# adeyemiadeoye/SelfConcordantSmoothOptimization.jl

Measured on AMD Instinct MI355X. Metric: iterate!() iterations/sec + achieved HBM GB/s, ProxGGNSCORE n=1M m=16k, higher is better.
Workload: dtype f64

## Files before the change

### selfconcordantsmoothoptimization.jl_amd/csrc/gram.hip

```cpp
#include <algorithm>
#include <cstdlib>
#include <type_traits>
#include <vector>

#include "common.h"

namespace scs {

}
#include "gram_strip.h"
namespace scs {

#define LDS_BARRIER()                                          \
  do {                                                         \
    asm volatile("s_waitcnt lgkmcnt(0)" ::: "memory");         \
    __builtin_amdgcn_s_barrier();                              \
    asm volatile("" ::: "memory");                             \
  } while (0)

__device__ __forceinline__ int bnd_claim(unsigned* ctr, int ntiles) {
  const int q8 = ntiles / 8, r8 = ntiles % 8;
  const int x0 = (int)((unsigned)__builtin_amdgcn_s_getreg((15 << 11) | 20) & 7u);
  for (int d = 0; d < 8; ++d) {
    const int x = (x0 + d) & 7, len = q8 + (x < r8 ? 1 : 0);
    if (len == 0) continue;
// ... 443 lines not shown
}

void gram_tile_list(int nb, int2* out, int* ntiles) {
  const int S = 8;
  const int nsb = (nb + S - 1) / S;
  int t = 0;
  for (int sbi = 0; sbi < nsb; ++sbi)
    for (int sbj = 0; sbj <= sbi; ++sbj)
      for (int i = sbi * S; i < (sbi + 1) * S && i < nb; ++i)
        for (int j = sbj * S; j < (sbj + 1) * S && j < nb; ++j)
          if (i >= j) out[t++] = make_int2(i, j);
  *ntiles = t;
}

void gram_tile_list_tall(int nb, int2* out, int* ntiles) {
  const int nbi = nb / 2, SI = 4, SJ = 8;
  int t = 0;
  for (int sbi = 0; sbi < (nbi + SI - 1) / SI; ++sbi)
    for (int sbj = 0; sbj <= sbi; ++sbj)
      for (int I = sbi * SI; I < (sbi + 1) * SI && I < nbi; ++I)
        for (int j = sbj * SJ; j < (sbj + 1) * SJ && j < nb; ++j)
          if (j <= 2 * I + 1) out[t++] = make_int2(I, j);
  *ntiles = t;
}

void gram_tile_list_rowmajor(int nb, int2* out) {
  int t = 0;
  for (int i = 0; i < nb; ++i)
    for (int j = 0; j <= i; ++j) out[t++] = make_int2(i, j);
}

hipError_t gram_launch_gen(const double* A1, int64_t lda1, const double* A2, int64_t lda2, const double* w,
                           int64_t k0, int64_t k1, const int2* tiles, int ntiles, double* G, int64_t ldg, int flags,
                           hipStream_t st);

template <int PIPE, int TI = 2, bool CM = false, bool AV = false, bool BND = false>
__global__ __launch_bounds__(128 * TI, (TI == 2 ? 2 : 1)) void gram_sia_kernel(
    const double* __restrict__ A, int64_t S, const double* __restrict__ w, int64_t k0, int64_t Nk,
// ... 12 lines not shown
    const int4* __restrict__ work, int seglen, int nsplit, double* __restrict__ P,
    const double* __restrict__ v, double* __restrict__ VP, int64_t vps, unsigned* __restrict__ scnt, int sob) {
  constexpr int PIPE = 1;
  constexpr bool CM = false, BND = false;
  const double* const A2 = nullptr;
  const int64_t S2 = 0;
#include "gram_sia_body.h"
}

static int env_int(const char* name, int dflt) {
  const char* e = getenv(name);
  return e ? atoi(e) : dflt;
}
int gram_sia_mode() {
  static const int v = env_int("SCS_GRAM_SIA", 1);
  return v;
}
int gram_tall_mode() {
  static const int v = env_int("SCS_GRAM_GLDS", 3);
  return v;
}

int gram_fuse_ok(int tall) {
  const char* e = getenv("SCS_GRAM_FUSE");
  const int mode = e ? atoi(e) : 1;
  if (mode == 0 || (!tall && mode < 2)) return 0;
  return tall ? gram_tall_mode() == 3 : gram_sia_mode() == 1;
}

__global__ void gram_vfinal_kernel(const double* __restrict__ VP, int npiece, int64_t vps, int64_t m,
                                   double* __restrict__ out) {
  const int64_t f = (int64_t)blockIdx.x * blockDim.x + threadIdx.x;
  if (f >= m) return;
  double s = VP[f];
  for (int p = 1; p < npiece; ++p) s += VP[(int64_t)p * vps + f];
  out[f] = s;
}

hipError_t gram_vfinal_launch(const double* VP, int npiece, int64_t vps, int64_t m, double* out, hipStream_t st) {
  hipLaunchKernelGGL(gram_vfinal_kernel, dim3((unsigned)((m + 255) / 256)), dim3(256), 0, st, VP, npiece, vps, m, out);
  return hipGetLastError();
}

static thread_local const char* g_main_name = "";
const char* gram_main_kernel_name() { return g_main_name; }

hipError_t gram_launch(const void* Av, int a32, int64_t lda, const double* w, int64_t Nk, const int2* tiles,
                       int ntiles, double* G, int64_t ldg, int packed, int tall, hipStream_t st, const double* v,
                       double* VP, int64_t vps) {
  if (ntiles <= 0) return hipSuccess;
  const int flags = ((packed & 1) ? GRAM_PACKED : GRAM_UPPER) | ((packed & 2) ? GRAM_ACCUMULATE : 0);
  if (v && !gram_fuse_ok(tall)) return hipErrorInvalidValue;
  if (a32) {
    const float* A = (const float*)Av;
    if (tall && v) {
      g_main_name = "gram_sia_ta_kernel<float, 4, true>";
      hipLaunchKernelGGL((gram_sia_ta_kernel<float, 4, true>), dim3(ntiles), dim3(512), 0, st, A, lda, w, (int64_t)0,
                         Nk, tiles, ntiles, G, ldg, flags, nullptr, 0, 0, nullptr, v, VP, vps, nullptr, 0);
    } else if (v) {
      g_main_name = "gram_sia_ta_kernel<float, 2, true>";
// ... 3 lines not shown
      g_main_name = "gram_sia_ta_kernel<float, 4, false>";
      hipLaunchKernelGGL((gram_sia_ta_kernel<float, 4, false>), dim3(ntiles), dim3(512), 0, st, A, lda, w, (int64_t)0,
                         Nk, tiles, ntiles, G, ldg, flags, nullptr, 0, 0, nullptr, nullptr, nullptr, (int64_t)0,
                         nullptr, 0);
    } else {
      g_main_name = "gram_sia_ta_kernel<float, 2, false>";
      hipLaunchKernelGGL((gram_sia_ta_kernel<float, 2, false>), dim3(ntiles), dim3(256), 0, st, A, lda, w, (int64_t)0,
                         Nk, tiles, ntiles, G, ldg, flags, nullptr, 0, 0, nullptr, nullptr, nullptr, (int64_t)0,
                         nullptr, 0);
    }
    return hipGetLastError();
  }
  const double* A = (const double*)Av;
  if (v) {
    if (tall) {
      g_main_name = "gram_sia_kernel<1, 4, false, true, false>";
      hipLaunchKernelGGL((gram_sia_kernel<1, 4, false, true>), dim3(ntiles), dim3(512), 0, st, A, lda, w, (int64_t)0,
                         Nk, tiles, ntiles, G, ldg, flags, nullptr, 0, 0, nullptr, v, VP, vps, nullptr, 0, nullptr, (int64_t)0);
    } else {
      g_main_name = "gram_sia_kernel<1, 2, false, true, false>";
      hipLaunchKernelGGL((gram_sia_kernel<1, 2, false, true>), dim3(ntiles), dim3(256), 0, st, A, lda, w, (int64_t)0,
                         Nk, tiles, ntiles, G, ldg, flags, nullptr, 0, 0, nullptr, v, VP, vps, nullptr, 0, nullptr, (int64_t)0);
    }
    return hipGetLastError();
  }
  if (!tall && gram_sia_mode() == 0) {
    g_main_name = "gram_f64_kernel<false, 2, true, false>";
    hipLaunchKernelGGL((gram_f64_kernel<false, 2, true>), dim3(ntiles), dim3(256), 0, st, A, lda, A, lda, w,
                       (int64_t)0, Nk, tiles, ntiles, G, ldg, flags, nullptr, 0, 0, nullptr);
  } else if (!tall) {
    g_main_name = "gram_sia_kernel<1, 2, false, false, false>";
    hipLaunchKernelGGL((gram_sia_kernel<1, 2>), dim3(ntiles), dim3(256), 0, st, A, lda, w, (int64_t)0, Nk, tiles,
                       ntiles, G, ldg, flags, nullptr, 0, 0, nullptr, nullptr, nullptr, (int64_t)0, nullptr, 0, nullptr, (int64_t)0);
  } else if (gram_tall_mode() == 3) {
    g_main_name = "gram_sia_kernel<1, 4, false, false, false>";
    hipLaunchKernelGGL((gram_sia_kernel<1, 4>), dim3(ntiles), dim3(512), 0, st, A, lda, w, (int64_t)0, Nk, tiles,
                       ntiles, G, ldg, flags, nullptr, 0, 0, nullptr, nullptr, nullptr, (int64_t)0, nullptr, 0, nullptr, (int64_t)0);
  } else {
    g_main_name = "gram_glds_kernel<true, 1>";
    hipLaunchKernelGGL((gram_glds_kernel<true, 1>), dim3(ntiles), dim3(512), 0, st, A, lda, A, lda, w, (int64_t)0, Nk,
                       tiles, ntiles, G, ldg, flags, nullptr, 0, 0, nullptr);
  }
  return hipGetLastError();
}

template <int QC>
__global__ __launch_bounds__(256) void gram_small_kernel(const double* __restrict__ A1, int64_t lda1,
                                                         const double* A2, int64_t lda2,
                                                         const double* __restrict__ w, int64_t k0, int64_t Nk,
                                                         const int2* __restrict__ tiles, double* G, int64_t ldg,
                                                         int flags) {
  constexpr int NQ = GT / QC;
// ... 125 lines not shown
                       ntiles, G, ldg, flags, nullptr, 0, 0, nullptr);
  return hipGetLastError();
}

template <int TI>
__global__ void gram_combine_kernel(const double* __restrict__ P, const int4* __restrict__ items, int nsplit,
                                    double* __restrict__ G, int64_t ldg, int packed) {
  constexpr int GTI = 64 * TI;
  const int4 it = items[blockIdx.y];
  for (int e = blockIdx.x * blockDim.x + threadIdx.x; e < GTI * GT; e += gridDim.x * blockDim.x) {
    const int jl = e / GTI, il = e % GTI;
    double sum = 0.0;
    for (int sp = 0; sp < nsplit; ++sp) sum += P[(int64_t)(it.w + sp) * GTI * GT + e];
    double* dst = (packed & 1) ? G + ((int64_t)it.z * (GTI / GT) + il / GT) * GT * GT + jl * GT + (il % GT)
                               : G + ((int64_t)it.x * GTI + il) * ldg + (int64_t)it.y * GT + jl;
    if (packed & 2) *dst += sum;
    else *dst = sum;
  }
}

hipError_t gram_launch_sched(const void* Av, int a32, int64_t lda, const double* w, int64_t Nk, const int4* work,
                             int seglen, int nsplit, const int4* comb, int ncomb, double* P, double* G, int64_t ldg,
                             int packed, int tall, hipStream_t st, const double* v, double* VP, int64_t vps,
                             unsigned* scnt, int sob) {
  const double* A = (const double*)Av;
  if (scnt && !(gram_fuse_ok(tall) || (tall ? gram_tall_mode() == 3 : gram_sia_mode() == 1)))
    return hipErrorInvalidValue;
  const int flags = ((packed & 1) ? GRAM_PACKED : GRAM_UPPER) | ((packed & 2) ? GRAM_ACCUMULATE : 0);
  const int glds = gram_tall_mode();
  if (v && !gram_fuse_ok(tall)) return hipErrorInvalidValue;
// ... 7 lines not shown
      g_main_name = "gram_sia_ta_kernel<float, 2, true>";
      hipLaunchKernelGGL((gram_sia_ta_kernel<float, 2, true>), dim3(8 * seglen), dim3(256), 0, st, Af, lda, w,
                         (int64_t)0, Nk, nullptr, 0, G, ldg, flags, work, seglen, nsplit, P, v, VP, vps, scnt, sob);
    } else if (tall) {
      g_main_name = "gram_sia_ta_kernel<float, 4, false>";
      hipLaunchKernelGGL((gram_sia_ta_kernel<float, 4, false>), dim3(8 * seglen), dim3(512), 0, st, Af, lda, w,
                         (int64_t)0, Nk, nullptr, 0, G, ldg, flags, work, seglen, nsplit, P, nullptr, nullptr,
                         (int64_t)0, scnt, sob);
    } else {
      g_main_name = "gram_sia_ta_kernel<float, 2, false>";
      hipLaunchKernelGGL((gram_sia_ta_kernel<float, 2, false>), dim3(8 * seglen), dim3(256), 0, st, Af, lda, w,
                         (int64_t)0, Nk, nullptr, 0, G, ldg, flags, work, seglen, nsplit, P, nullptr, nullptr,
                         (int64_t)0, scnt, sob);
    }
  } else if (v && tall) {
    g_main_name = "gram_sia_kernel<1, 4, false, true, false>";
    hipLaunchKernelGGL((gram_sia_kernel<1, 4, false, true>), dim3(8 * seglen), dim3(512), 0, st, A, lda, w,
                       (int64_t)0, Nk, nullptr, 0, G, ldg, flags, work, seglen, nsplit, P, v, VP, vps, scnt, sob, nullptr, (int64_t)0);
  } else if (v) {
    g_main_name = "gram_sia_kernel<1, 2, false, true, false>";
    hipLaunchKernelGGL((gram_sia_kernel<1, 2, false, true>), dim3(8 * seglen), dim3(256), 0, st, A, lda, w,
                       (int64_t)0, Nk, nullptr, 0, G, ldg, flags, work, seglen, nsplit, P, v, VP, vps, scnt, sob, nullptr, (int64_t)0);
  } else if (tall && glds == 3) {
    g_main_name = "gram_sia_kernel<1, 4, false, false, false>";
    hipLaunchKernelGGL((gram_sia_kernel<1, 4>), dim3(8 * seglen), dim3(512), 0, st, A, lda, w, (int64_t)0, Nk,
                       nullptr, 0, G, ldg, flags, work, seglen, nsplit, P, nullptr, nullptr, (int64_t)0, scnt, sob, nullptr, (int64_t)0);
  } else if (tall && glds == 2) {
    g_main_name = "gram_glds_kernel<true, 1>";
    hipLaunchKernelGGL((gram_glds_kernel<true, 1>), dim3(8 * seglen), dim3(512), 0, st, A, lda, A, lda, w, (int64_t)0,
                       Nk, nullptr, 0, G, ldg, flags, work, seglen, nsplit, P);
  } else if (tall && glds == 1) {
    g_main_name = "gram_glds_kernel<true, 0>";
    hipLaunchKernelGGL(gram_glds_kernel<true>, dim3(8 * seglen), dim3(512), 0, st, A, lda, A, lda, w, (int64_t)0, Nk,
                       nullptr, 0, G, ldg, flags, work, seglen, nsplit, P);
  } else if (tall) {
    g_main_name = "gram_f64_kernel<false, 4, true, false>";
    hipLaunchKernelGGL((gram_f64_kernel<false, 4, true>), dim3(8 * seglen), dim3(512), 0, st, A, lda, A, lda, w,
                       (int64_t)0, Nk, nullptr, 0, G, ldg, flags, work, seglen, nsplit, P);
  } else if (gram_sia_mode() == 1) {
    g_main_name = "gram_sia_kernel<1, 2, false, false, false>";
    hipLaunchKernelGGL((gram_sia_kernel<1, 2>), dim3(8 * seglen), dim3(256), 0, st, A, lda, w, (int64_t)0, Nk, nullptr,
// ... 57 lines not shown
  int S = 1;
  if (tail_max > 0 && 4 * tail_max < 3 * slots_per_xcd)
    S = std::max(2, std::min(16, slots_per_xcd / tail_max));
  std::vector<std::vector<int4>> seg(8);
  comb.clear();
  int pslot = 0, t0 = 0;
  for (int x = 0; x < 8; ++x) {
    const int n = q + (x < r ? 1 : 0);
    const int tail = (S > 1) ? n % slots_per_xcd : 0;
    for (int i = 0; i < n - tail; ++i) {
      const int2 tl = tiles[t0 + i];
      seg[x].push_back(make_int4(tl.x, tl.y, -1, t0 + i));
    }
    if (diag_first_gti > 0)
      std::stable_partition(seg[x].begin(), seg[x].end(), [&](const int4& it) {
        return it.x == (int)((int64_t)it.y * GT / diag_first_gti);
      });
    for (int i = n - tail; i < n; ++i) {
      const int2 tl = tiles[t0 + i];
      comb.push_back(make_int4(tl.x, tl.y, t0 + i, pslot));
      for (int sp = 0; sp < S; ++sp) seg[x].push_back(make_int4(tl.x, tl.y, sp, pslot + sp));
      pslot += S;
    }
    t0 += n;
  }
  size_t seglen = 0;
  for (auto& v : seg) seglen = std::max(seglen, v.size());
  work.assign(8 * seglen, make_int4(-1, -1, -1, -1));
  for (int x = 0; x < 8; ++x)
    for (size_t i = 0; i < seg[x].size(); ++i) work[x * seglen + i] = seg[x][i];
  *nsplit = S;
// ... 13 lines not shown
```

### selfconcordantsmoothoptimization.jl_amd/csrc/gram_sia_body.h

```cpp
  static_assert(!(AV && CM), "the fused Aᵀv runs on the panel-blocked A only");
  static_assert(!CM || sizeof(TA) == sizeof(double), "column-major operands are fp64");
  constexpr int GTI = 64 * TI;
  constexpr int NT = 128 * TI;
  constexpr int FS = NT / 8;
  constexpr int NTI = 4;
  constexpr int NA = GTI / FS;
  constexpr int NB = GT / FS;
  constexpr int NMM = 2 * NTI * 4;
  constexpr int NRD = NTI + 4;
  constexpr int TAIL = NMM / 4;
  const int packed = flags & GRAM_PACKED, accumulate = flags & GRAM_ACCUMULATE, upper = flags & GRAM_UPPER;
  __shared__ __attribute__((aligned(16))) double lds[(GTI + GT) * GBK];
  const int orig = blockIdx.x;
  const int xcd = orig % 8;
  int bi, bj, tix, part = -1, piece = 0;
  __shared__ int s_claim;
  if constexpr (BND) {
    tix = bnd_first(scnt, (unsigned)sob, ntiles, &s_claim);
    if (tix < 0 || tix >= ntiles) return;
    bi = tiles[tix].x;
    bj = tiles[tix].y;
  } else if (work) {
    const int4 it = work[xcd * seglen + orig / 8];
    if (it.x < 0) return;
    bi = it.x;
    bj = it.y;
    tix = it.w;
// ... 1 lines not shown
      piece = it.z;
      const int64_t L = ((Nk - k0 + (int64_t)nsplit * GBK - 1) / ((int64_t)nsplit * GBK)) * GBK;
      part = it.w;
      k0 = k0 + it.z * L;
      Nk = k0 + L < Nk ? k0 + L : Nk;
      if (Nk < k0) Nk = k0;
    }
  } else {
    const int q8 = ntiles / 8, r8 = ntiles % 8;
    tix = (xcd < r8 ? xcd * (q8 + 1) : r8 * (q8 + 1) + (xcd - r8) * q8) + orig / 8;
    const int2 tl = tiles[tix];
    bi = tl.x;
    bj = tl.y;
  }
bnd_tile:
  int tid_ = threadIdx.x;
  if constexpr (BND) asm volatile("" : "+v"(tid_));
  const int tid = tid_, lane = tid & 63, wid = tid >> 6;
  const int wr = wid >> 1, wc = wid & 1;
  const int sc = tid & 7, sf0 = tid >> 3;
  const int64_t st0 = k0 / GBK;
  const TA* srcA = CM ? A + ((int64_t)bi * GTI + sf0) * S + k0 + 2 * sc
                      : A + ((int64_t)bi * (GTI / GT) * S + st0) * GT * GBK + sf0 * GBK + 2 * sc;
  const TA* B2 = (CM && A2) ? (const TA*)A2 : A;
  const int64_t SB2 = (CM && A2) ? S2 : S;
  const TA* srcB = CM ? B2 + ((int64_t)bj * GT + sf0) * SB2 + k0 + 2 * sc
                      : A + ((int64_t)bj * S + st0) * GT * GBK + sf0 * GBK + 2 * sc;
  const double* srcW = w + k0 + 2 * sc;
  const double* srcV = AV ? v + k0 + 2 * sc : nullptr;
  double* la = lds;
  double* lb = lds + GTI * GBK;
  int woff[NA];
#pragma unroll
  for (int i = 0; i < NA; ++i) {
    const int f = sf0 + FS * i;
    woff[i] = f * GBK + 2 * (sc ^ swz(f));
  }
  typedef typename pair_of<TA>::type PR;
  PR ra[NA], rb[NB];
  v2d rw, rv;
  double av[NB];
#pragma unroll
  for (int i = 0; i < NB; ++i) av[i] = 0.0;
  auto gload = [&](int64_t st, auto fa) {
    constexpr bool FA = decltype(fa)::value;
    if (PIPE == 3 && st >= 2) return;
    if (CM) {
#pragma unroll
      for (int i = 0; i < NA; ++i) ra[i] = *(const PR*)(srcA + st * GBK + (int64_t)FS * i * S);
#pragma unroll
      for (int i = 0; i < NB; ++i) rb[i] = *(const PR*)(srcB + st * GBK + (int64_t)FS * i * SB2);
    } else {
      const int64_t so = st * GT * GBK;
#pragma unroll
      for (int i = 0; i < NA; ++i) {
        const int f = FS * i;
        ra[i] = *(const PR*)(srcA + so + (f >> 7) * S * GT * GBK + (f & 127) * GBK);
      }
#pragma unroll
      for (int i = 0; i < NB; ++i) rb[i] = *(const PR*)(srcB + so + FS * GBK * i);
    }
    rw = *(const v2d*)(srcW + st * GBK);
    if (FA) rv = *(const v2d*)(srcV + st * GBK);
  };
  auto swrite = [&](auto fa) {
    constexpr bool FA = decltype(fa)::value;
#pragma unroll
    for (int i = 0; i < NA; ++i) *(v2d*)(la + woff[i]) = widen(ra[i]);
#pragma unroll
    for (int i = 0; i < NB; ++i) *(v2d*)(lb + woff[i]) = widen(rb[i]) * rw;
    if (FA) {
#pragma unroll
      for (int i = 0; i < NB; ++i) {
        const v2d b = widen(rb[i]);
        av[i] = __builtin_fma(b[1], rv[1], __builtin_fma(b[0], rv[0], av[i]));
      }
    }
  };
  const int fl = lane & 15, g = lane >> 4, s = swz(fl);
  struct Frag {
    v2d a[NTI], b[4];
  };
  auto fread = [&](int p, Frag& F) {
    const int pc = ((4 * p + g) ^ s) * 2;
#pragma unroll
    for (int t = 0; t < NTI; ++t) F.a[t] = *(const v2d*)(la + (wr * 64 + 16 * t + fl) * GBK + pc);
#pragma unroll
    for (int t = 0; t < 4; ++t) F.b[t] = *(const v2d*)(lb + (wc * 64 + 16 * t + fl) * GBK + pc);
  };
  v4d acc[NTI][4];
#pragma unroll
  for (int i = 0; i < NTI; ++i)
#pragma unroll
    for (int j = 0; j < 4; ++j) acc[i][j] = (v4d){0.0, 0.0, 0.0, 0.0};
  auto mm = [&](const Frag& F, int n0, int n1) {
#pragma unroll
    for (int n = n0; n < n1; ++n) {
      const int u = n / (4 * NTI), ti = (n / 4) % NTI, tj = n & 3;
      acc[ti][tj] = __builtin_amdgcn_mfma_f64_16x16x4f64(F.a[ti][u], F.b[tj][u], acc[ti][tj], 0, 0, 0);
    }
  };
  auto barrier = [&]() {
    __builtin_amdgcn_sched_barrier(0);
    __builtin_amdgcn_s_waitcnt(0xC07F);
    __builtin_amdgcn_s_barrier();
    asm volatile("" ::: "memory");
    __builtin_amdgcn_sched_barrier(0);
  };
  const int nk = (int)((Nk - k0) / GBK);
  Frag F0, F1;
  auto run = [&](auto fa) {
    if (nk > 0) {
      gload(0, fa);
      swrite(fa);
      if (nk > 1) gload(1, fa);
      barrier();
      fread(0, F0);
    }
    auto body = [&](int k, bool has1, bool has2) {
      __builtin_amdgcn_sched_barrier(0);
      fread(1, F1);
      mm(F0, 0, NMM);
      if (PIPE) {
#pragma unroll
        for (int i = 0; i < NRD; ++i) {
          __builtin_amdgcn_sched_group_barrier(0x008, NMM / NRD, 0);
          __builtin_amdgcn_sched_group_barrier(0x100, 1, 0);
        }
      }
      barrier();
      if (has1) swrite(fa);
      if (has2) gload(k + 2, fa);
      mm(F1, 0, NMM - TAIL);
      if (PIPE) {
        if (has1) {
#pragma unroll
          for (int i = 0; i < NA + NB; ++i) {
            __builtin_amdgcn_sched_group_barrier(0x008, (NMM - TAIL) / (NA + NB), 0);
            __builtin_amdgcn_sched_group_barrier(0x200, 1, 0);
            if (has2) __builtin_amdgcn_sched_group_barrier(0x020, 1, 0);
          }
        }
        __builtin_amdgcn_sched_group_barrier(0x008, NMM, 0);
      }
      if (has1) {
        barrier();
        fread(0, F0);
      }
      mm(F1, NMM - TAIL, NMM);
      if (PIPE && has1) {
#pragma unroll
        for (int i = 0; i < NRD; ++i) {
          __builtin_amdgcn_sched_group_barrier(0x008, TAIL / NRD > 0 ? TAIL / NRD : 1, 0);
          __builtin_amdgcn_sched_group_barrier(0x100, 1, 0);
        }
      }
    };
    int k = 0;
    for (; k + 2 < nk; ++k) body(k, true, true);
    if (k + 1 < nk) {
      body(k, true, false);
      ++k;
    }
    if (k < nk) body(k, false, false);
  };
  const bool dav = AV && (int64_t)bj * GT / GTI == bi;
  if constexpr (AV) {
    if (dav) run(std::true_type{});
    else run(std::false_type{});
  } else {
    run(std::false_type{});
  }

  if (dav) {
#pragma unroll
    for (int i = 0; i < NB; ++i) {
      double t = av[i];
      t += __shfl_xor(t, 1);
      t += __shfl_xor(t, 2);
      t += __shfl_xor(t, 4);
      if (sc == 0) VP[(int64_t)piece * vps + (int64_t)bj * GT + sf0 + FS * i] = t;
    }
  }

  if constexpr (BND || CM) {
#pragma unroll
    for (int ti = 0; ti < NTI; ++ti)
      gram_tile_store_row(acc[ti], ti, wr, wc, g, fl, part, P, GTI, packed, upper, accumulate, G, ldg, tix, bi, bj);
  } else {
#pragma unroll
    for (int ti = 0; ti < NTI; ++ti)
#pragma unroll
      for (int tj = 0; tj < 4; ++tj)
#pragma unroll
        for (int r = 0; r < 4; ++r) {
          const int il = wr * 64 + 16 * ti + g + 4 * r;
          const int jl = wc * 64 + 16 * tj + fl;
          double* dst;
          if (part >= 0) {
            P[((int64_t)part * GT + jl) * GTI + il] = acc[ti][tj][r];
            continue;
          }
          if (packed) dst = G + ((int64_t)tix * (GTI / GT) + il / GT) * GT * GT + jl * GT + (il % GT);
          else if (upper) dst = G + ((int64_t)bi * GTI + il) * ldg + (int64_t)bj * GT + jl;
          else dst = G + ((int64_t)bj * GT + jl) * ldg + (int64_t)bi * GTI + il;
          if (accumulate) *dst += acc[ti][tj][r];
          else *dst = acc[ti][tj][r];
        }
  }
  if (!BND && scnt && part < 0) {
    __threadfence();
    __syncthreads();
    if (tid == 0) atomicAdd(scnt + bj / sob, 1u);
  }
  if constexpr (BND) {
    tix = bnd_next(scnt, ntiles, &s_claim);
    if (tix >= ntiles) return;
    bi = tiles[tix].x;
    bj = tiles[tix].y;
    goto bnd_tile;
// ... 2 lines not shown
```

### selfconcordantsmoothoptimization.jl_amd/csrc/kernels.h

```cpp
#pragma once
#include <hip/hip_runtime.h>
#include <stdint.h>

#include <vector>
#include "../../include/scsopt.h"

namespace scs {

struct ProxArgsH {
  int reg = 0;
  int use_prox = 1;
  double lam = 0.0, lam2 = 0.0;
  const double* lb = nullptr;
  const double* ub = nullptr;
  const int* gstart = nullptr;
  const int* gend = nullptr;
  const double* gw = nullptr;
  int ngroups = 0;
  const int* gmap = nullptr;
};

void gram_tile_list(int nb, int2* out, int* ntiles);
void gram_tile_list_tall(int nb, int2* out, int* ntiles);
const char* gram_main_kernel_name();
hipError_t gram_launch(const void* A, int a32, int64_t lda, const double* w, int64_t Nk, const int2* tiles, int ntiles,
                       double* G, int64_t ldg, int packed, int tall, hipStream_t st, const double* v = nullptr,
                       double* VP = nullptr, int64_t vps = 0);
int gram_fuse_ok(int tall);
hipError_t gram_vfinal_launch(const double* VP, int npiece, int64_t vps, int64_t m, double* out, hipStream_t st);
void gram_tile_list_rowmajor(int nb, int2* out);
hipError_t gram_launch_gen(const double* A1, int64_t lda1, const double* A2, int64_t lda2, const double* w,
                           int64_t k0, int64_t k1, const int2* tiles, int ntiles, double* G, int64_t ldg, int flags,
                           hipStream_t st);
hipError_t gram_launch_work_cm(const double* A1, int64_t lda1, const double* A2, int64_t lda2, const double* w,
                               int64_t K, const int4* work, int seglen, int nsplit, double* P, hipStream_t st);
hipError_t gram_launch_bounded(const double* A1, int64_t lda1, const double* A2, int64_t lda2, const double* w,
                               int64_t k0, int64_t k1, const int2* tiles, int ntiles, double* G, int64_t ldg, int flags,
                               unsigned* ctr, unsigned skip, int slots, hipStream_t st, bool zeroed = false);
// ... 295 lines not shown
```

### selfconcordantsmoothoptimization.jl_amd/csrc/scsopt.cpp

```cpp
#include <hip/hip_runtime.h>
#include <rccl/rccl.h>

#include <dlfcn.h>
#include <execinfo.h>
#include <signal.h>

#include <algorithm>
#include <chrono>
#include <cmath>
#include <cstdarg>
#include <cstddef>
#include <cstdio>
#include <cstdlib>
#include <cstring>
#include <limits>
#include <atomic>
#include <condition_variable>
#include <functional>
#include <memory>
#include <mutex>
#include <string>
#include <thread>
#include <utility>
#include <vector>
// ... 155 lines not shown
  double *zpart = nullptr, *z = nullptr, *gN = nullptr, *hN = nullptr, *wN = nullptr, *vN = nullptr,
         *valpart = nullptr;
  int nval = 1;
  int nchunk = 1;
  double* tpart = nullptr;
  double *G = nullptr, *Gc = nullptr;
  int2* tiles = nullptr;
  int ntiles = 0;
  int tall = 0;
  int2* utiles = nullptr;
  int nslots = 0;
  int4* gwork = nullptr;
  int4* gcomb = nullptr;
  int gseglen = 0, gncomb = 0, gnsplit = 1;
  double* gpart = nullptr;
  double* vpart = nullptr;
  struct GStrip {
    int4* work = nullptr;
    int4* comb = nullptr;
    int seglen = 0, nsplit = 1, ncomb = 0;
  };
  std::vector<GStrip> gstrip;
  GStrip gpipe;
  std::vector<unsigned> gp_target;
  unsigned* gp_cnt = nullptr;
  int* gp_flag = nullptr;
  int vpieces = 1;
  hipStream_t sf = nullptr;
  std::vector<hipEvent_t> evstrip;
  hipEvent_t evfac = nullptr;
// ... 393 lines not shown
  if (c->tall) {
    gram_tile_list_tall(nb, tl.data(), &nt);
    ul.resize(2 * (size_t)nt);
    for (int t = 0; t < nt; ++t) {
      ul[2 * t] = make_int2(2 * tl[t].x, tl[t].y);
      ul[2 * t + 1] = make_int2(2 * tl[t].x + 1, tl[t].y);
    }
  } else {
    gram_tile_list(nb, tl.data(), &nt);
    ul.assign(tl.begin(), tl.begin() + nt);
  }
  c->tiles = dalloc<int2>(c, nt);
  HCK(hipMemcpyAsync(c->tiles, tl.data(), sizeof(int2) * nt, hipMemcpyHostToDevice, c->st));
  c->ntiles = nt;
  c->nslots = (int)ul.size();
  {
    const char* ev = std::getenv("SCS_GRAM_SCHED");
    if (!(ev && ev[0] == '0')) {
      std::vector<int4> wk, cb;
      int npart = 0;
      const char* df = std::getenv("SCS_GRAM_DIAGFIRST");
      const int dfg = (df && df[0] == '0') ? 0 : c->tall ? 256 : (df && df[0] == '1') ? 128 : 0;
      c->gseglen = gram_schedule(tl.data(), nt, 32 * (c->tall ? 1 : 2), wk, cb, &c->gnsplit, &npart, dfg);
      c->gncomb = (int)cb.size();
      c->gwork = dalloc<int4>(c, wk.size());
      HCK(hipMemcpyAsync(c->gwork, wk.data(), sizeof(int4) * wk.size(), hipMemcpyHostToDevice, c->st));
      if (c->gncomb > 0) {
        c->gcomb = dalloc<int4>(c, cb.size());
        HCK(hipMemcpyAsync(c->gcomb, cb.data(), sizeof(int4) * cb.size(), hipMemcpyHostToDevice, c->st));
        c->gpart = dalloc<double>(c, (size_t)npart * (c->tall ? 256 : 128) * 128);
      }
    }
  }
  {
    const int OB = chol_outer_block(), ns = (nb + OB - 1) / OB;
    c->gstrip.assign(ns, scs_ctx::GStrip());
    c->vpieces = std::max(c->gnsplit, 1);
    int npart_max = 0;
    for (int s2 = 0; s2 < ns; ++s2) {
      std::vector<int2> st;
      for (int t = 0; t < nt; ++t)
        if (tl[t].y / OB == s2) st.push_back(tl[t]);
      std::vector<int4> wk, cb;
      int nsplit = 1, npart = 0;
      scs_ctx::GStrip& g = c->gstrip[s2];
      g.seglen = gram_schedule(st.data(), (int)st.size(), 32 * (c->tall ? 1 : 2), wk, cb, &nsplit, &npart);
      g.nsplit = nsplit;
      g.ncomb = (int)cb.size();
      g.work = dalloc<int4>(c, wk.size());
      HCK(hipMemcpyAsync(g.work, wk.data(), sizeof(int4) * wk.size(), hipMemcpyHostToDevice, c->st));
      if (!cb.empty()) {
        g.comb = dalloc<int4>(c, cb.size());
// ... 909 lines not shown
    c->ring_r0[0] = c->ring_r0[1] = -1;
  }
  const int64_t R = c->ring_rows;
  const int64_t nchunk = ceil_div(std::max<int64_t>(c->N, 1), R);
  for (int64_t k = 0; k < nchunk; ++k) {
    const int s = (int)(k & 1);
    double* slot = c->ringA + (size_t)s * R * c->mpad;
    const int64_t r0 = k * R, n = std::min(R, c->N - r0);
    if (c->ring_r0[s] >= 0)
      HCK(launch_densify_range(c->rowptr, c->colidx, c->val, c->sp_f32, c->ring_r0[s], c->ring_n[s], R, 1, slot, c->st));
    HCK(launch_densify_range(c->rowptr, c->colidx, c->val, c->sp_f32, r0, n, R, 0, slot, c->st));
    c->ring_r0[s] = r0;
    c->ring_n[s] = n;
    const int mode = packed | (k > 0 ? 2 : 0);
    const int64_t nk = round_up(std::max<int64_t>(n, 1), 16);
    if (c->gwork)
      HCK(gram_launch_sched(slot, 0, R / 16, w + r0, nk, c->gwork, c->gseglen, c->gnsplit, c->gcomb, c->gncomb, c->gpart,
                            out, c->mpad, mode, c->tall, c->st));
    else
      HCK(gram_launch(slot, 0, R / 16, w + r0, nk, c->tiles, c->ntiles, out, c->mpad, mode, c->tall, c->st));
    c->gram_kname = gram_main_kernel_name();
  }
}

void gram_main(scs_ctx* c, const double* w, double* out, int packed, const double* v = nullptr,
               double* vout = nullptr) {
  if (sparse_gram(c)) {
    if (v) fail(c, SCS_ERR_ARG, "internal: the sparse Gram forms no Aᵀv");
    gram_sparse(c, w, out, packed);
    return;
  }
  if (sparse_streams(c)) {
    if (v) fail(c, SCS_ERR_ARG, "internal: the streaming sparse Gram forms no Aᵀv");
    gram_main_stream(c, w, out, packed);
    return;
  }
  const double* A = dense_A(c);
  const int npiece = (v && c->gwork) ? std::max(c->gnsplit, 1) : 1;
  if (v && npiece > 1) HCK(hipMemsetAsync(c->vpart, 0, sizeof(double) * npiece * c->mpad, c->st));
  if (c->gwork)
    HCK(gram_launch_sched(A, dense_a32(c), c->nstage, w, c->Npad, c->gwork, c->gseglen, c->gnsplit, c->gcomb, c->gncomb,
                          c->gpart, out, c->mpad, packed, c->tall, c->st, v, c->vpart, c->mpad));
  else
    HCK(gram_launch(A, dense_a32(c), c->nstage, w, c->Npad, c->tiles, c->ntiles, out, c->mpad, packed, c->tall, c->st,
                    v, c->vpart, c->mpad));
  c->gram_kname = gram_main_kernel_name();
  if (v) HCK(gram_vfinal_launch(c->vpart, npiece, c->mpad, c->m, vout, c->st));
}

bool gram_x_independent(const scs_ctx* c) {
  if (c->loss != SCS_LOSS_LEAST_SQUARES) return false;
  return c->method == SCS_PROX_NSCORE || (c->method == SCS_PROX_GGNSCORE && c->ggn == SCS_GGN_LINEAR_LS);
}

void gram_and_reduce(scs_ctx* c, const double* w, const double* v, double* vec_dev) {
  ensure_gram(c);
  ensure_red(c);
  hipEvent_t e0;
  const bool cacheable = c->gram_cache && gram_x_independent(c);
  const size_t gbytes = sizeof(double) * (size_t)c->mpad * c->mpad;
// ... 721 lines not shown
  dfree_t(c, c->cbstage);
  ++c->data_gen;
  c->nnz = 0;
  dfree_t(c, c->y);
  dfree_t(c, c->G);
  dfree_t(c, c->Gc);
  dfree_t(c, c->tiles);
  dfree_t(c, c->utiles);
  for (double** v : {&c->At, &c->Ps, &c->Ms, &c->bS, &c->uN, &c->hvec, &c->hg}) dfree_t(c, *v);
  dfree_t(c, c->stiles);
  c->n1pad = 0;
  c->NpS = 0;
  c->nstiles = 0;
  dfree_t(c, c->gwork);
  dfree_t(c, c->gcomb);
  dfree_t(c, c->gpart);
  dfree_t(c, c->vpart);
  for (auto& g : c->gstrip) {
    dfree_t(c, g.work);
    dfree_t(c, g.comb);
  }
  c->gstrip.clear();
  c->vpieces = 1;
  c->gseglen = c->gncomb = 0;
  c->gnsplit = 1;
  dfree_t(c, c->W);
  dfree_t(c, c->ysol);
  dfree_t(c, c->trilist);
  dfree_t(c, c->cinfo);
  dfree_t(c, c->lsbuf);
// ... 2113 lines not shown
```

Before: 0.2566.

## Pair odd diagonal Gram blocks into one tall tile and tune MFMA scheduling

In the tall 256x128 Gram kernel, the tiles that cover an odd diagonal block are now paired, so one workgroup computes two diagonal 128x128 blocks from two A panels. The B operand is the weighted A panel itself, which avoids loading it separately. A new paired tile list and schedule are built and used for non-packed Gram output, and the combine and Aᵀv reduction paths are updated for the pair encoding. Separately, new kernel PIPE variants (10 by default) reorder the sched_group_barrier interleaving of MFMA, LDS and global operations. This is meant to remove wasted work on the diagonal half-tiles and to improve instruction overlap, at the cost of more complex indexing and extra schedule state.

```diff
diff --git a/selfconcordantsmoothoptimization.jl_amd/csrc/gram.hip b/selfconcordantsmoothoptimization.jl_amd/csrc/gram.hip
--- a/selfconcordantsmoothoptimization.jl_amd/csrc/gram.hip
+++ b/selfconcordantsmoothoptimization.jl_amd/csrc/gram.hip
@@ -1,4 +1,5 @@
 #include <algorithm>
+#include <cstdio>
 #include <cstdlib>
 #include <type_traits>
 #include <vector>
@@ -9,6 +10,7 @@
 
 }
 #include "gram_strip.h"
+#include "gram_tiles.h"
 namespace scs {
 
 #define LDS_BARRIER()                                          \
@@ -482,14 +484,10 @@
 }
 
 void gram_tile_list_tall(int nb, int2* out, int* ntiles) {
-  const int nbi = nb / 2, SI = 4, SJ = 8;
-  int t = 0;
-  for (int sbi = 0; sbi < (nbi + SI - 1) / SI; ++sbi)
-    for (int sbj = 0; sbj <= sbi; ++sbj)
-      for (int I = sbi * SI; I < (sbi + 1) * SI && I < nbi; ++I)
-        for (int j = sbj * SJ; j < (sbj + 1) * SJ && j < nb; ++j)
-          if (j <= 2 * I + 1) out[t++] = make_int2(I, j);
-  *ntiles = t;
+  *ntiles = gram_tile_list_tall_t(nb, false, out, [](int x, int y) { return make_int2(x, y); });
+}
+void gram_tile_list_tall_paired(int nb, int2* out, int* ntiles) {
+  *ntiles = gram_tile_list_tall_t(nb, true, out, [](int x, int y) { return make_int2(x, y); });
 }
 
 void gram_tile_list_rowmajor(int nb, int2* out) {
@@ -532,11 +530,20 @@
 }
 int gram_sia_mode() {
   static const int v = env_int("SCS_GRAM_SIA", 1);
-  return v;
+  return v >= 8 ? 1 : v;
+}
+constexpr int GRAM_EDGE_DEFAULT = 2;
+int gram_edge_bits() {
+  static const int v = env_int("SCS_GRAM_SIA", 1);
+  return v >= 8 && v <= 15 ? (v & 7) : GRAM_EDGE_DEFAULT;
 }
 int gram_tall_mode() {
   static const int v = env_int("SCS_GRAM_GLDS", 3);
   return v;
+}
+int gram_pair_ok() {
+  static const int v = env_int("SCS_GRAM_DIAGPAIR", 1);
+  return v != 0 && gram_tall_mode() == 3;
 }
 
 int gram_fuse_ok(int tall) {
@@ -562,6 +569,19 @@
 
 static thread_local const char* g_main_name = "";
 const char* gram_main_kernel_name() { return g_main_name; }
+
+template <bool AV, class... Args>
+static void sia_tall_launch(unsigned grid, hipStream_t st, Args... args) {
+  static thread_local char name[64];
+  int pipe = 1;
+  switch (gram_edge_bits()) {
+    case 2: pipe = 10; hipLaunchKernelGGL((gram_sia_kernel<10, 4, false, AV>), dim3(grid), dim3(512), 0, st, args...); break;
+    case 4: pipe = 12; hipLaunchKernelGGL((gram_sia_kernel<12, 4, false, AV>), dim3(grid), dim3(512), 0, st, args...); break;
+    default: hipLaunchKernelGGL((gram_sia_kernel<1, 4, false, AV>), dim3(grid), dim3(512), 0, st, args...);
+  }
+  snprintf(name, sizeof(name), "gram_sia_kernel<%d, 4, false, %s, false>", pipe, AV ? "true" : "false");
+  g_main_name = name;
+}
 
 hipError_t gram_launch(const void* Av, int a32, int64_t lda, const double* w, int64_t Nk, const int2* tiles,
                        int ntiles, double* G, int64_t ldg, int packed, int tall, hipStream_t st, const double* v,
@@ -595,9 +615,9 @@
   const double* A = (const double*)Av;
   if (v) {
     if (tall) {
-      g_main_name = "gram_sia_kernel<1, 4, false, true, false>";
-      hipLaunchKernelGGL((gram_sia_kernel<1, 4, false, true>), dim3(ntiles), dim3(512), 0, st, A, lda, w, (int64_t)0,
-                         Nk, tiles, ntiles, G, ldg, flags, nullptr, 0, 0, nullptr, v, VP, vps, nullptr, 0, nullptr, (int64_t)0);
+      sia_tall_launch<true>((unsigned)ntiles, st, A, lda, w, (int64_t)0, Nk, tiles, ntiles, G, ldg, flags,
+                            (const int4*)nullptr, 0, 0, (double*)nullptr, v, VP, vps, (unsigned*)nullptr, 0,
+                            (const double*)nullptr, (int64_t)0);
     } else {
       g_main_name = "gram_sia_kernel<1, 2, false, true, false>";
       hipLaunchKernelGGL((gram_sia_kernel<1, 2, false, true>), dim3(ntiles), dim3(256), 0, st, A, lda, w, (int64_t)0,
@@ -614,9 +634,9 @@
     hipLaunchKernelGGL((gram_sia_kernel<1, 2>), dim3(ntiles), dim3(256), 0, st, A, lda, w, (int64_t)0, Nk, tiles,
                        ntiles, G, ldg, flags, nullptr, 0, 0, nullptr, nullptr, nullptr, (int64_t)0, nullptr, 0, nullptr, (int64_t)0);
   } else if (gram_tall_mode() == 3) {
-    g_main_name = "gram_sia_kernel<1, 4, false, false, false>";
-    hipLaunchKernelGGL((gram_sia_kernel<1, 4>), dim3(ntiles), dim3(512), 0, st, A, lda, w, (int64_t)0, Nk, tiles,
-                       ntiles, G, ldg, flags, nullptr, 0, 0, nullptr, nullptr, nullptr, (int64_t)0, nullptr, 0, nullptr, (int64_t)0);
+    sia_tall_launch<false>((unsigned)ntiles, st, A, lda, w, (int64_t)0, Nk, tiles, ntiles, G, ldg, flags,
+                           (const int4*)nullptr, 0, 0, (double*)nullptr, (const double*)nullptr, (double*)nullptr,
+                           (int64_t)0, (unsigned*)nullptr, 0, (const double*)nullptr, (int64_t)0);
   } else {
     g_main_name = "gram_glds_kernel<true, 1>";
     hipLaunchKernelGGL((gram_glds_kernel<true, 1>), dim3(ntiles), dim3(512), 0, st, A, lda, A, lda, w, (int64_t)0, Nk,
@@ -772,6 +792,11 @@
     for (int sp = 0; sp < nsplit; ++sp) sum += P[(int64_t)(it.w + sp) * GTI * GT + e];
     double* dst = (packed & 1) ? G + ((int64_t)it.z * (GTI / GT) + il / GT) * GT * GT + jl * GT + (il % GT)
                                : G + ((int64_t)it.x * GTI + il) * ldg + (int64_t)it.y * GT + jl;
+    if (TI == 4 && gram_item_is_pair(it.y)) {
+      int bi, bj;
+      gram_item_block(it.x, it.y, il / GT, &bi, &bj);
+      dst = G + ((int64_t)bi * GT + il % GT) * ldg + (int64_t)bj * GT + jl;
+    }
     if (packed & 2) *dst += sum;
     else *dst = sum;
   }
@@ -809,17 +834,16 @@
                          (int64_t)0, scnt, sob);
     }
   } else if (v && tall) {
-    g_main_name = "gram_sia_kernel<1, 4, false, true, false>";
-    hipLaunchKernelGGL((gram_sia_kernel<1, 4, false, true>), dim3(8 * seglen), dim3(512), 0, st, A, lda, w,
-                       (int64_t)0, Nk, nullptr, 0, G, ldg, flags, work, seglen, nsplit, P, v, VP, vps, scnt, sob, nullptr, (int64_t)0);
+    sia_tall_launch<true>((unsigned)(8 * seglen), st, A, lda, w, (int64_t)0, Nk, (const int2*)nullptr, 0, G, ldg, flags,
+                          work, seglen, nsplit, P, v, VP, vps, scnt, sob, (const double*)nullptr, (int64_t)0);
   } else if (v) {
     g_main_name = "gram_sia_kernel<1, 2, false, true, false>";
     hipLaunchKernelGGL((gram_sia_kernel<1, 2, false, true>), dim3(8 * seglen), dim3(256), 0, st, A, lda, w,
                        (int64_t)0, Nk, nullptr, 0, G, ldg, flags, work, seglen, nsplit, P, v, VP, vps, scnt, sob, nullptr, (int64_t)0);
   } else if (tall && glds == 3) {
-    g_main_name = "gram_sia_kernel<1, 4, false, false, false>";
-    hipLaunchKernelGGL((gram_sia_kernel<1, 4>), dim3(8 * seglen), dim3(512), 0, st, A, lda, w, (int64_t)0, Nk,
-                       nullptr, 0, G, ldg, flags, work, seglen, nsplit, P, nullptr, nullptr, (int64_t)0, scnt, sob, nullptr, (int64_t)0);
+    sia_tall_launch<false>((unsigned)(8 * seglen), st, A, lda, w, (int64_t)0, Nk, (const int2*)nullptr, 0, G, ldg,
+                           flags, work, seglen, nsplit, P, (const double*)nullptr, (double*)nullptr, (int64_t)0, scnt,
+                           sob, (const double*)nullptr, (int64_t)0);
   } else if (tall && glds == 2) {
     g_main_name = "gram_glds_kernel<true, 1>";
     hipLaunchKernelGGL((gram_glds_kernel<true, 1>), dim3(8 * seglen), dim3(512), 0, st, A, lda, A, lda, w, (int64_t)0,
@@ -907,7 +931,7 @@
     }
     if (diag_first_gti > 0)
       std::stable_partition(seg[x].begin(), seg[x].end(), [&](const int4& it) {
-        return it.x == (int)((int64_t)it.y * GT / diag_first_gti);
+        return gram_item_designated(it.x, it.y, diag_first_gti);
       });
     for (int i = n - tail; i < n; ++i) {
       const int2 tl = tiles[t0 + i];
diff --git a/selfconcordantsmoothoptimization.jl_amd/csrc/gram_sia_body.h b/selfconcordantsmoothoptimization.jl_amd/csrc/gram_sia_body.h
--- a/selfconcordantsmoothoptimization.jl_amd/csrc/gram_sia_body.h
+++ b/selfconcordantsmoothoptimization.jl_amd/csrc/gram_sia_body.h
@@ -9,8 +9,12 @@
   constexpr int NMM = 2 * NTI * 4;
   constexpr int NRD = NTI + 4;
   constexpr int TAIL = NMM / 4;
+  constexpr bool E1 = PIPE >= 8 && (PIPE & 1), E2 = PIPE >= 8 && (PIPE & 2), E3 = PIPE >= 8 && (PIPE & 4);
+  constexpr bool PAIRT = TI == 4 && !CM && !BND;
+  constexpr int LBR = PAIRT ? GTI : GT;
+  constexpr int NAV = PAIRT ? NA : NB;
   const int packed = flags & GRAM_PACKED, accumulate = flags & GRAM_ACCUMULATE, upper = flags & GRAM_UPPER;
-  __shared__ __attribute__((aligned(16))) double lds[(GTI + GT) * GBK];
+  __shared__ __attribute__((aligned(16))) double lds[(GTI + LBR) * GBK];
   const int orig = blockIdx.x;
   const int xcd = orig % 8;
   int bi, bj, tix, part = -1, piece = 0;
@@ -42,6 +46,15 @@
     bj = tl.y;
   }
 bnd_tile:
+  int pa = (GTI / GT) * bi, pb = pa + 1;
+  bool pair = false;
+  if constexpr (PAIRT) {
+    if (gram_item_is_pair(bj)) {
+      pair = true;
+      gram_item_panels(bi, bj, &pa, &pb);
+      bj = pa;
+    }
+  }
   int tid_ = threadIdx.x;
   if constexpr (BND) asm volatile("" : "+v"(tid_));
   const int tid = tid_, lane = tid & 63, wid = tid >> 6;
@@ -49,7 +62,8 @@
   const int sc = tid & 7, sf0 = tid >> 3;
   const int64_t st0 = k0 / GBK;
   const TA* srcA = CM ? A + ((int64_t)bi * GTI + sf0) * S + k0 + 2 * sc
-                      : A + ((int64_t)bi * (GTI / GT) * S + st0) * GT * GBK + sf0 * GBK + 2 * sc;
+                      : A + ((int64_t)pa * S + st0) * GT * GBK + sf0 * GBK + 2 * sc;
+  const int64_t pd = (int64_t)(pb - pa) * S * GT * GBK;
   const TA* B2 = (CM && A2) ? (const TA*)A2 : A;
   const int64_t SB2 = (CM && A2) ? S2 : S;
   const TA* srcB = CM ? B2 + ((int64_t)bj * GT + sf0) * SB2 + k0 + 2 * sc
@@ -67,11 +81,11 @@
   typedef typename pair_of<TA>::type PR;
   PR ra[NA], rb[NB];
   v2d rw, rv;
-  double av[NB];
-#pragma unroll
-  for (int i = 0; i < NB; ++i) av[i] = 0.0;
-  auto gload = [&](int64_t st, auto fa) {
-    constexpr bool FA = decltype(fa)::value;
+  double av[NAV];
+#pragma unroll
+  for (int i = 0; i < NAV; ++i) av[i] = 0.0;
+  auto gload = [&](int64_t st, auto fa, auto pt) {
+    constexpr bool FA = decltype(fa)::value, PT = decltype(pt)::value;
     if (PIPE == 3 && st >= 2) return;
     if (CM) {
 #pragma unroll
@@ -83,18 +97,32 @@
 #pragma unroll
       for (int i = 0; i < NA; ++i) {
         const int f = FS * i;
-        ra[i] = *(const PR*)(srcA + so + (f >> 7) * S * GT * GBK + (f & 127) * GBK);
-      }
-#pragma unroll
-      for (int i = 0; i < NB; ++i) rb[i] = *(const PR*)(srcB + so + FS * GBK * i);
+        ra[i] = *(const PR*)(srcA + so + (f >> 7) * pd + (f & 127) * GBK);
+      }
+      if (!PT) {
+#pragma unroll
+        for (int i = 0; i < NB; ++i) rb[i] = *(const PR*)(srcB + so + FS * GBK * i);
+      }
     }
     rw = *(const v2d*)(srcW + st * GBK);
     if (FA) rv = *(const v2d*)(srcV + st * GBK);
   };
-  auto swrite = [&](auto fa) {
-    constexpr bool FA = decltype(fa)::value;
+  auto swrite = [&](auto fa, auto pt) {
+    constexpr bool FA = decltype(fa)::value, PT = decltype(pt)::value;
 #pragma unroll
     for (int i = 0; i < NA; ++i) *(v2d*)(la + woff[i]) = widen(ra[i]);
+    if constexpr (PT) {
+#pragma unroll
+      for (int i = 0; i < NA; ++i) *(v2d*)(lb + woff[i]) = widen(ra[i]) * rw;
+      if (FA) {
+#pragma unroll
+        for (int i = 0; i < NAV; ++i) {
+          const v2d b = widen(ra[i]);
+          av[i] = __builtin_fma(b[1], rv[1], __builtin_fma(b[0], rv[0], av[i]));
+        }
+      }
+      return;
+    }
 #pragma unroll
     for (int i = 0; i < NB; ++i) *(v2d*)(lb + woff[i]) = widen(rb[i]) * rw;
     if (FA) {
@@ -106,6 +134,7 @@
     }
   };
   const int fl = lane & 15, g = lane >> 4, s = swz(fl);
+  const int brow = wc * 64 + (pair ? (wr >> 1) * GT : 0);
   struct Frag {
     v2d a[NTI], b[4];
   };
@@ -114,7 +143,7 @@
 #pragma unroll
     for (int t = 0; t < NTI; ++t) F.a[t] = *(const v2d*)(la + (wr * 64 + 16 * t + fl) * GBK + pc);
 #pragma unroll
-    for (int t = 0; t < 4; ++t) F.b[t] = *(const v2d*)(lb + (wc * 64 + 16 * t + fl) * GBK + pc);
+    for (int t = 0; t < 4; ++t) F.b[t] = *(const v2d*)(lb + (brow + 16 * t + fl) * GBK + pc);
   };
   v4d acc[NTI][4];
 #pragma unroll
@@ -137,11 +166,12 @@
   };
   const int nk = (int)((Nk - k0) / GBK);
   Frag F0, F1;
-  auto run = [&](auto fa) {
+  auto run = [&](auto fa, auto pt) {
+    constexpr int NW = decltype(pt)::value ? 2 * NA : NA + NB;
     if (nk > 0) {
-      gload(0, fa);
-      swrite(fa);
-      if (nk > 1) gload(1, fa);
+      gload(0, fa, pt);
+      swrite(fa, pt);
+      if (nk > 1) gload(1, fa, pt);
       barrier();
       fread(0, F0);
     }
@@ -152,21 +182,28 @@
       if (PIPE) {
 #pragma unroll
         for (int i = 0; i < NRD; ++i) {
-          __builtin_amdgcn_sched_group_barrier(0x008, NMM / NRD, 0);
+          if (!E1) __builtin_amdgcn_sched_group_barrier(0x008, NMM / NRD, 0);
           __builtin_amdgcn_sched_group_barrier(0x100, 1, 0);
+          if (E1) __builtin_amdgcn_sched_group_barrier(0x008, NMM / NRD, 0);
         }
       }
       barrier();
-      if (has1) swrite(fa);
-      if (has2) gload(k + 2, fa);
+      if (has1) swrite(fa, pt);
+      if (has2) gload(k + 2, fa, pt);
       mm(F1, 0, NMM - TAIL);
       if (PIPE) {
         if (has1) {
-#pragma unroll
-          for (int i = 0; i < NA + NB; ++i) {
-            __builtin_amdgcn_sched_group_barrier(0x008, (NMM - TAIL) / (NA + NB), 0);
+          constexpr int HEAD = E2 ? NMM / NRD : 0, Q = (NMM - TAIL - HEAD) / NW;
+          if (E2) {
+            __builtin_amdgcn_sched_group_barrier(0x008, HEAD, 0);
+            __builtin_amdgcn_sched_group_barrier(0x002, 64, 0);
+          }
+#pragma unroll
+          for (int i = 0; i < NW; ++i) {
+            if (!E3) __builtin_amdgcn_sched_group_barrier(0x008, Q, 0);
             __builtin_amdgcn_sched_group_barrier(0x200, 1, 0);
             if (has2) __builtin_amdgcn_sched_group_barrier(0x020, 1, 0);
+            if (E3) __builtin_amdgcn_sched_group_barrier(0x008, Q, 0);
           }
         }
         __builtin_amdgcn_sched_group_barrier(0x008, NMM, 0);
@@ -192,25 +229,34 @@
     }
     if (k < nk) body(k, false, false);
   };
-  const bool dav = AV && (int64_t)bj * GT / GTI == bi;
-  if constexpr (AV) {
-    if (dav) run(std::true_type{});
-    else run(std::false_type{});
+  const bool dav = AV && (pair || (int64_t)bj * GT / GTI == bi);
+  if constexpr (PAIRT) {
+    if (pair) run(std::bool_constant<AV>{}, std::true_type{});
+    else if (dav) run(std::bool_constant<AV>{}, std::false_type{});
+    else run(std::false_type{}, std::false_type{});
+  } else if constexpr (AV) {
+    if (dav) run(std::true_type{}, std::false_type{});
+    else run(std::false_type{}, std::false_type{});
   } else {
-    run(std::false_type{});
+    run(std::false_type{}, std::false_type{});
   }
 
   if (dav) {
 #pragma unroll
-    for (int i = 0; i < NB; ++i) {
+    for (int i = 0; i < NAV; ++i) {
+      if (i >= NB && !pair) continue;
       double t = av[i];
       t += __shfl_xor(t, 1);
       t += __shfl_xor(t, 2);
       t += __shfl_xor(t, 4);
-      if (sc == 0) VP[(int64_t)piece * vps + (int64_t)bj * GT + sf0 + FS * i] = t;
+      const int64_t row = i < NB ? (int64_t)bj * GT + sf0 + FS * i : (int64_t)pb * GT + sf0 + FS * (i - NB);
+      if (sc == 0) VP[(int64_t)piece * vps + row] = t;
     }
   }
 
+  const int pw = (wr >> 1) ? pb : pa;
+  const int64_t grow = pair ? (int64_t)(pw - (wr >> 1)) * GT : (int64_t)bi * GTI;
+  const int64_t gcol = pair ? (int64_t)pw * GT : (int64_t)bj * GT;
   if constexpr (BND || CM) {
 #pragma unroll
     for (int ti = 0; ti < NTI; ++ti)
@@ -230,8 +276,8 @@
             continue;
           }
           if (packed) dst = G + ((int64_t)tix * (GTI / GT) + il / GT) * GT * GT + jl * GT + (il % GT);
-          else if (upper) dst = G + ((int64_t)bi * GTI + il) * ldg + (int64_t)bj * GT + jl;
-          else dst = G + ((int64_t)bj * GT + jl) * ldg + (int64_t)bi * GTI + il;
+          else if (upper) dst = G + (grow + il) * ldg + gcol + jl;
+          else dst = G + (gcol + jl) * ldg + grow + il;
           if (accumulate) *dst += acc[ti][tj][r];
           else *dst = acc[ti][tj][r];
         }
diff --git a/selfconcordantsmoothoptimization.jl_amd/csrc/gram_tiles.h b/selfconcordantsmoothoptimization.jl_amd/csrc/gram_tiles.h
--- /dev/null
+++ b/selfconcordantsmoothoptimization.jl_amd/csrc/gram_tiles.h
@@ -0,0 +1,59 @@
+#pragma once
+
+#if defined(__HIPCC__)
+#define SCS_TILES_HD __host__ __device__
+#else
+#define SCS_TILES_HD
+#endif
+
+namespace scs {
+
+SCS_TILES_HD inline bool gram_item_is_pair(int y) { return y < 0; }
+SCS_TILES_HD inline int gram_pair_encode(int I2) { return -1 - I2; }
+SCS_TILES_HD inline int gram_pair_second(int y) { return -1 - y; }
+
+SCS_TILES_HD inline void gram_item_panels(int x, int y, int* pa, int* pb) {
+  if (gram_item_is_pair(y)) {
+    *pa = 2 * x + 1;
+    *pb = 2 * gram_pair_second(y) + 1;
+  } else {
+    *pa = 2 * x;
+    *pb = 2 * x + 1;
+  }
+}
+
+SCS_TILES_HD inline void gram_item_block(int x, int y, int h, int* bi, int* bj) {
+  if (gram_item_is_pair(y)) {
+    *bi = *bj = 2 * (h ? gram_pair_second(y) : x) + 1;
+  } else {
+    *bi = 2 * x + h;
+    *bj = y;
+  }
+}
+
+SCS_TILES_HD inline bool gram_item_designated(int x, int y, int gti) {
+  return gram_item_is_pair(y) || x == (int)((long long)y * 128 / gti);
+}
+
+template <class T2, class Make>
+inline int gram_tile_list_tall_t(int nb, bool pair, T2* out, Make make) {
+  const int nbi = nb / 2, SI = 4, SJ = 8;
+  int t = 0;
+  for (int sbi = 0; sbi < (nbi + SI - 1) / SI; ++sbi)
+    for (int sbj = 0; sbj <= sbi; ++sbj)
+      for (int I = sbi * SI; I < (sbi + 1) * SI && I < nbi; ++I)
+        for (int j = sbj * SJ; j < (sbj + 1) * SJ && j < nb; ++j) {
+          if (j > 2 * I + 1) continue;
+          if (pair && j == 2 * I + 1) {
+            if (I % 2 == 1) continue;
+            if (I + 1 < nbi) {
+              out[t++] = make(I, gram_pair_encode(I + 1));
+              continue;
+            }
+          }
+          out[t++] = make(I, j);
+        }
+  return t;
+}
+
+}
diff --git a/selfconcordantsmoothoptimization.jl_amd/csrc/kernels.h b/selfconcordantsmoothoptimization.jl_amd/csrc/kernels.h
--- a/selfconcordantsmoothoptimization.jl_amd/csrc/kernels.h
+++ b/selfconcordantsmoothoptimization.jl_amd/csrc/kernels.h
@@ -22,6 +22,8 @@
 
 void gram_tile_list(int nb, int2* out, int* ntiles);
 void gram_tile_list_tall(int nb, int2* out, int* ntiles);
+void gram_tile_list_tall_paired(int nb, int2* out, int* ntiles);
+int gram_pair_ok();
 const char* gram_main_kernel_name();
 hipError_t gram_launch(const void* A, int a32, int64_t lda, const double* w, int64_t Nk, const int2* tiles, int ntiles,
                        double* G, int64_t ldg, int packed, int tall, hipStream_t st, const double* v = nullptr,
diff --git a/selfconcordantsmoothoptimization.jl_amd/csrc/scsopt.cpp b/selfconcordantsmoothoptimization.jl_amd/csrc/scsopt.cpp
--- a/selfconcordantsmoothoptimization.jl_amd/csrc/scsopt.cpp
+++ b/selfconcordantsmoothoptimization.jl_amd/csrc/scsopt.cpp
@@ -193,6 +193,11 @@
   int4* gcomb = nullptr;
   int gseglen = 0, gncomb = 0, gnsplit = 1;
   double* gpart = nullptr;
+  int2* ptiles = nullptr;
+  int nptiles = 0;
+  int4* pwork = nullptr;
+  int4* pcomb = nullptr;
+  int pseglen = 0, pncomb = 0, pnsplit = 1;
   double* vpart = nullptr;
   struct GStrip {
     int4* work = nullptr;
@@ -616,11 +621,21 @@
   HCK(hipMemcpyAsync(c->tiles, tl.data(), sizeof(int2) * nt, hipMemcpyHostToDevice, c->st));
   c->ntiles = nt;
   c->nslots = (int)ul.size();
+  std::vector<int2> tp;
+  if (c->tall && gram_pair_ok()) {
+    int np = 0;
+    tp.resize(tl.size());
+    gram_tile_list_tall_paired(nb, tp.data(), &np);
+    tp.resize(np);
+    c->ptiles = dalloc<int2>(c, np);
+    HCK(hipMemcpyAsync(c->ptiles, tp.data(), sizeof(int2) * np, hipMemcpyHostToDevice, c->st));
+    c->nptiles = np;
+  }
   {
     const char* ev = std::getenv("SCS_GRAM_SCHED");
     if (!(ev && ev[0] == '0')) {
       std::vector<int4> wk, cb;
-      int npart = 0;
+      int npart = 0, npartp = 0;
       const char* df = std::getenv("SCS_GRAM_DIAGFIRST");
       const int dfg = (df && df[0] == '0') ? 0 : c->tall ? 256 : (df && df[0] == '1') ? 128 : 0;
       c->gseglen = gram_schedule(tl.data(), nt, 32 * (c->tall ? 1 : 2), wk, cb, &c->gnsplit, &npart, dfg);
@@ -630,14 +645,25 @@
       if (c->gncomb > 0) {
         c->gcomb = dalloc<int4>(c, cb.size());
         HCK(hipMemcpyAsync(c->gcomb, cb.data(), sizeof(int4) * cb.size(), hipMemcpyHostToDevice, c->st));
-        c->gpart = dalloc<double>(c, (size_t)npart * (c->tall ? 256 : 128) * 128);
       }
+      if (c->ptiles) {
+        c->pseglen = gram_schedule(tp.data(), c->nptiles, 32, wk, cb, &c->pnsplit, &npartp, dfg);
+        c->pncomb = (int)cb.size();
+        c->pwork = dalloc<int4>(c, wk.size());
+        HCK(hipMemcpyAsync(c->pwork, wk.data(), sizeof(int4) * wk.size(), hipMemcpyHostToDevice, c->st));
+        if (c->pncomb > 0) {
+          c->pcomb = dalloc<int4>(c, cb.size());
+          HCK(hipMemcpyAsync(c->pcomb, cb.data(), sizeof(int4) * cb.size(), hipMemcpyHostToDevice, c->st));
+        }
+      }
+      if (std::max(npart, npartp) > 0)
+        c->gpart = dalloc<double>(c, (size_t)std::max(npart, npartp) * (c->tall ? 256 : 128) * 128);
     }
   }
   {
     const int OB = chol_outer_block(), ns = (nb + OB - 1) / OB;
     c->gstrip.assign(ns, scs_ctx::GStrip());
-    c->vpieces = std::max(c->gnsplit, 1);
+    c->vpieces = std::max(std::max(c->gnsplit, c->pnsplit), 1);
     int npart_max = 0;
     for (int s2 = 0; s2 < ns; ++s2) {
       std::vector<int2> st;
@@ -1577,11 +1603,14 @@
     c->ring_n[s] = n;
     const int mode = packed | (k > 0 ? 2 : 0);
     const int64_t nk = round_up(std::max<int64_t>(n, 1), 16);
+    const bool pr = c->ptiles && !(packed & 1);
     if (c->gwork)
-      HCK(gram_launch_sched(slot, 0, R / 16, w + r0, nk, c->gwork, c->gseglen, c->gnsplit, c->gcomb, c->gncomb, c->gpart,
-                            out, c->mpad, mode, c->tall, c->st));
+      HCK(gram_launch_sched(slot, 0, R / 16, w + r0, nk, pr ? c->pwork : c->gwork, pr ? c->pseglen : c->gseglen,
+                            pr ? c->pnsplit : c->gnsplit, pr ? c->pcomb : c->gcomb, pr ? c->pncomb : c->gncomb,
+                            c->gpart, out, c->mpad, mode, c->tall, c->st));
     else
-      HCK(gram_launch(slot, 0, R / 16, w + r0, nk, c->tiles, c->ntiles, out, c->mpad, mode, c->tall, c->st));
+      HCK(gram_launch(slot, 0, R / 16, w + r0, nk, pr ? c->ptiles : c->tiles, pr ? c->nptiles : c->ntiles, out,
+                      c->mpad, mode, c->tall, c->st));
     c->gram_kname = gram_main_kernel_name();
   }
 }
@@ -1599,14 +1628,17 @@
     return;
   }
   const double* A = dense_A(c);
-  const int npiece = (v && c->gwork) ? std::max(c->gnsplit, 1) : 1;
+  const bool pr = c->ptiles && !(packed & 1);
+  const int nsplit = pr ? c->pnsplit : c->gnsplit;
+  const int npiece = (v && c->gwork) ? std::max(nsplit, 1) : 1;
   if (v && npiece > 1) HCK(hipMemsetAsync(c->vpart, 0, sizeof(double) * npiece * c->mpad, c->st));
   if (c->gwork)
-    HCK(gram_launch_sched(A, dense_a32(c), c->nstage, w, c->Npad, c->gwork, c->gseglen, c->gnsplit, c->gcomb, c->gncomb,
+    HCK(gram_launch_sched(A, dense_a32(c), c->nstage, w, c->Npad, pr ? c->pwork : c->gwork,
+                          pr ? c->pseglen : c->gseglen, nsplit, pr ? c->pcomb : c->gcomb, pr ? c->pncomb : c->gncomb,
                           c->gpart, out, c->mpad, packed, c->tall, c->st, v, c->vpart, c->mpad));
   else
-    HCK(gram_launch(A, dense_a32(c), c->nstage, w, c->Npad, c->tiles, c->ntiles, out, c->mpad, packed, c->tall, c->st,
-                    v, c->vpart, c->mpad));
+    HCK(gram_launch(A, dense_a32(c), c->nstage, w, c->Npad, pr ? c->ptiles : c->tiles, pr ? c->nptiles : c->ntiles,
+                    out, c->mpad, packed, c->tall, c->st, v, c->vpart, c->mpad));
   c->gram_kname = gram_main_kernel_name();
   if (v) HCK(gram_vfinal_launch(c->vpart, npiece, c->mpad, c->m, vout, c->st));
 }
@@ -2358,6 +2390,11 @@
   c->nstiles = 0;
   dfree_t(c, c->gwork);
   dfree_t(c, c->gcomb);
+  dfree_t(c, c->ptiles);
+  dfree_t(c, c->pwork);
+  dfree_t(c, c->pcomb);
+  c->nptiles = c->pseglen = c->pncomb = 0;
+  c->pnsplit = 1;
   dfree_t(c, c->gpart);
   dfree_t(c, c->vpart);
   for (auto& g : c->gstrip) {
```

Result: faster. 0.2595, median of 6 (+1.1%).
